# Tongji-MIC-Lab/TDVC

Hardware: AMD Instinct MI355X
Metric: 1080p P-frames/sec (encode + reconstruct, lambda=2048 config) (higher is better)
Workload: dtype f16; 1 GPU; 1x 1920x1080 (padded 1088x1920) 7-frame synthetic GOP (seed 1234), batch 1, P-frames coded in GOP order; gop=7, batch=1, parallelism=gop-sharded x1, weights=closed-form filler (no checkpoint ships)

## Files before the change

### include/tdvc_hip.h

```cpp
#ifndef TDVC_HIP_H
#define TDVC_HIP_H

#include <stdint.h>

#ifdef __cplusplus
extern "C" {
#endif

#define TDVC_OK 0
#define TDVC_EINVAL (-1)
#define TDVC_ENOSUP (-2)

typedef struct {
  void* p;
  int32_t N, H, W, C;
  int64_t sn;
  int32_t sp;
  int32_t dtype;
} tdvc_fmap;

enum { TDVC_F16 = 0, TDVC_F32 = 1 };
enum { TDVC_ACT_NONE = 0, TDVC_ACT_RELU = 1, TDVC_ACT_LRELU = 2, TDVC_ACT_CLAMP01 = 3, TDVC_ACT_SIGMOID = 4 };
enum { TDVC_GDN_NONE = 0, TDVC_GDN_FWD = 1, TDVC_GDN_INV = 2 };
enum { TDVC_OUT_NHWC = 0,
// ... 43 lines not shown
int tdvc_conv_plan(int cin, int kh, int kw, int stride);
int64_t tdvc_conv_packed_bytes(int cout, int cin, int ntaps, int ck);
int tdvc_pack_conv_weights(const float* w_oihw, int cout, int cin_real, int cin, int kh, int kw,
                           int ntaps, const int8_t* tap_dy, const int8_t* tap_dx, int ck, uint16_t* dst);
int tdvc_conv2d(const tdvc_conv_desc* d, void* stream);
int tdvc_conv_chan_sum_rows(const tdvc_conv_desc* d);
int tdvc_conv_flow_supported(const tdvc_conv_desc* d);
const char* tdvc_conv_select(const tdvc_conv_desc* d);
int tdvc_conv2d_f32(const tdvc_conv_desc* d, void* stream);

typedef struct {
  tdvc_fmap x, y;
  const void* w;
  const float* bias;
  int32_t act1; float slope1;
  int32_t act2; float slope2;
  int32_t add_input;
  tdvc_fmap res2;
} tdvc_conv_pair_desc;
int64_t tdvc_conv_pair_packed_bytes(void);
int tdvc_pack_conv_pair_weights(const float* w1_oihw, const float* w2_oihw, uint16_t* dst);
int tdvc_conv_pair_supported(const tdvc_conv_pair_desc* d);
int tdvc_conv_pair(const tdvc_conv_pair_desc* d, void* stream);

typedef struct {
  tdvc_fmap x, om, y;
  const void* w;
  const float* bias;
  int32_t groups;
  int32_t act; float slope; int32_t round_before_act;
  void* x_planar;
} tdvc_dcn_desc;
int tdvc_dcn_fused(const tdvc_dcn_desc* d, void* stream);

int tdvc_dcn_v2_forward_f32(const float* input, const float* weight, const float* bias,
                            const float* offset, const float* mask, float* output,
                            int B, int C, int H, int W, int Cout,
                            int kh, int kw, int sh, int sw, int ph, int pw, int dh, int dw,
                            int deformable_group, void* stream);
int tdvc_dcn_v2_backward_f32(const float* input, const float* weight, const float* bias,
                             const float* offset, const float* mask, const float* grad_output,
                             float* grad_input, float* grad_offset, float* grad_mask,
                             float* grad_weight, float* grad_bias, float* columns,
                             int B, int C, int H, int W, int Cout,
                             int kh, int kw, int sh, int sw, int ph, int pw, int dh, int dw,
                             int deformable_group, void* stream);
// ... 219 lines not shown
```

### tdvc_amd/_lib.py

```python
from __future__ import annotations

import ctypes as C
import os

_HERE = os.path.dirname(os.path.abspath(__file__))
LIB_PATH = os.path.join(_HERE, "libtdvc_hip.so")

MAX_TAPS = 49
F16, F32 = 0, 1
ACT_NONE, ACT_RELU, ACT_LRELU, ACT_CLAMP01, ACT_SIGMOID = 0, 1, 2, 3, 4
GDN_NONE, GDN_FWD, GDN_INV = 0, 1, 2
OUT_NHWC, OUT_SHUFFLE2, OUT_NCHW_F32 = 0, 1, 2


class FMapDesc(C.Structure):
    _fields_ = [("p", C.c_void_p), ("N", C.c_int32), ("H", C.c_int32), ("W", C.c_int32), ("C", C.c_int32),
                ("sn", C.c_int64), ("sp", C.c_int32), ("dtype", C.c_int32)]


class ConvDesc(C.Structure):
    _fields_ = [("x", FMapDesc), ("y", FMapDesc), ("w", C.c_void_p), ("bias", C.c_void_p),
                ("cout", C.c_int32), ("ntaps", C.c_int32),
                ("tap_dy", C.c_int8 * MAX_TAPS), ("tap_dx", C.c_int8 * MAX_TAPS),
                ("kh", C.c_int32), ("kw", C.c_int32), ("stride", C.c_int32), ("pad", C.c_int32),
                ("ck", C.c_int32), ("square_input", C.c_int32), ("gdn", C.c_int32),
                ("aux", FMapDesc), ("act", C.c_int32), ("slope", C.c_float),
                ("round_before_act", C.c_int32), ("res", FMapDesc), ("res2", FMapDesc), ("out_mode", C.c_int32), ("s2d", C.c_int32),
                ("bcast_T", C.c_int32), ("bcast_slope", C.c_float), ("chan_sum", C.c_void_p), ("flow", FMapDesc)]


class DcnDesc(C.Structure):
    _fields_ = [("x", FMapDesc), ("om", FMapDesc), ("y", FMapDesc), ("w", C.c_void_p), ("bias", C.c_void_p),
                ("groups", C.c_int32), ("act", C.c_int32), ("slope", C.c_float), ("round_before_act", C.c_int32), ("x_planar", C.c_void_p)]


class ConvPairDesc(C.Structure):
    _fields_ = [("x", FMapDesc), ("y", FMapDesc), ("w", C.c_void_p), ("bias", C.c_void_p), ("act1", C.c_int32), ("slope1", C.c_float),
                ("act2", C.c_int32), ("slope2", C.c_float), ("add_input", C.c_int32), ("res2", FMapDesc)]


class WgradReduceJob(C.Structure):
    _fields_ = [("work", C.c_void_p), ("bwork", C.c_void_p), ("row_off", C.c_void_p), ("chan_off", C.c_void_p), ("tap_off", C.c_void_p),
                ("bias_index", C.c_void_p), ("dw", C.c_void_p), ("db", C.c_void_p), ("scale", C.c_float),
                ("nworkers", C.c_int32), ("cow", C.c_int32), ("ciw", C.c_int32), ("ntaps", C.c_int32), ("cout", C.c_int32), ("cin", C.c_int32),
                ("wblocks", C.c_int32), ("nblocks", C.c_int32)]


_P = C.c_void_p
_FM = C.POINTER(FMapDesc)


class CdfTablesDesc(C.Structure):
    _fields_ = [("cdfs", _P), ("sizes", _P), ("offsets", _P), ("stride", C.c_int32), ("ncdfs", C.c_int32)]


class CdfTablesDevDesc(C.Structure):
    _fields_ = [("cdf16", _P), ("starts", _P), ("sizes", _P), ("offsets", _P), ("n16", C.c_int32), ("ncdfs", C.c_int32)]


class ArLoopDesc(C.Structure):
    _fields_ = [("y_hat", FMapDesc), ("params", FMapDesc), ("x1", FMapDesc), ("pc", FMapDesc), ("gp", FMapDesc),
# ... 75 lines not shown
    "tdvc_rans_encode_lanes_dev_ref": (_i, [_ENC, _CDF]),
    "tdvc_ar_last_loop_launches": (_i64, []),
    "tdvc_ssim_level_work_floats": (_i64, [_i] * 5),
    "tdvc_ssim_level": (_i, [_P, _P, _i, _i, _i, _i, _P, _i, _f, _f, _P, _P, _P, _i64, _P]),
    "tdvc_avgpool2_pad_f32": (_i, [_P, _i64, _i, _i, _P, _P]),
    "tdvc_ssim_level_backward": (_i, [_P, _P, _i, _i, _i, _i, _P, _i, _f, _f, _P, _P, _f, _P, _P, _P]),
    "tdvc_msssim_level_grads": (_i, [_P, _P, _P, _i, _i, _P, _P, _P, _P, _P]),
    "tdvc_dcn_col2im_work_floats": (_i64, [_i, _i, _i, _i]),
    "tdvc_dcn_col2im": (_i, [_FM, _FM, _FM, _i, _P, _FM, _P, _i64, _P]),
    "tdvc_dcn_col2im_det": (_i, [_FM, _FM, _FM, _i, _P, _FM, _P, _i64, _P, _P, _P, _i, _P]),
    "tdvc_dcn_far_apply": (_i, [_P, _P, _P, _i, _P, _P]),
    "tdvc_conv_wgrad_work_floats": (_i64, [_i] * 6),
    "tdvc_conv_wgrad": (_i, [_FM, _FM] + [_i] * 6 + [_P] * 5 + [_i, _f, _P, _P, _i64, _P]),
    "tdvc_conv_wgrad_bias": (_i, [_FM, _FM] + [_i] * 6 + [_P] * 5 + [_i, _f, _P, _P, _P, _P, _i64, _P]),
    "tdvc_conv_wgrad_partials": (_i, [_FM, _FM] + [_i] * 6 + [_P] * 5 + [_i, _f, _P, _P, _P, _P, _i64, C.POINTER(WgradReduceJob), _P]),
    "tdvc_wgrad_reduce_batch": (_i, [_P, _P, _i, _i, _P]),
    "tdvc_gdn_backward": (_i, [_FM, _FM, _FM, _i, _FM, _FM, _P]),
    "tdvc_mul2_accumulate": (_i, [_FM, _FM, _FM, _P]),
    "tdvc_dcn_fused": (_i, [C.POINTER(DcnDesc), _P]),
    "tdvc_conv_pair_packed_bytes": (_i64, []),
    "tdvc_pack_conv_pair_weights": (_i, [_P, _P, _P]),
    "tdvc_conv_pair_supported": (_i, [C.POINTER(ConvPairDesc)]),
    "tdvc_conv_pair": (_i, [C.POINTER(ConvPairDesc), _P]),
    "tdvc_dcn_v2_forward_f32": (_i, [_P] * 6 + [_i] * 14 + [_P]),
    "tdvc_dcn_v2_backward_f32": (_i, [_P] * 12 + [_i] * 14 + [_P]),
    "tdvc_nchw_to_fmap": (_i, [_P, _i, _FM, _P]),
    "tdvc_fmap_to_nchw": (_i, [_FM, _i, _P, _P]),
    "tdvc_scale_act_res": (_i, [_FM, _P, _i, _f, _FM, _f, _FM, _FM, _P]),
    "tdvc_add_flow": (_i, [_FM, _FM, _P]),
    "tdvc_bcast_add_act": (_i, [_FM, _FM, _i, _f, _P]),
    "tdvc_channel_sum": (_i, [_FM, _P, _i, _P]),
    "tdvc_se_gate": (_i, [_P, _i, _f, _i, _i, _i, _P, _P, _P, _P, _P, _P]),
    "tdvc_upsample2x": (_i, [_FM, _FM, _P]),
    "tdvc_avgpool2": (_i, [_FM, _FM, _P]),
    "tdvc_spynet_level_input": (_i, [_FM, _FM, _FM, _FM, _FM, _P]),
    "tdvc_resize_bilinear": (_i, [_FM, _FM, _P, _P]),
    "tdvc_avgpool_k_work_floats": (_i64, [_i, _i, _i, _i, _i]),
    "tdvc_avgpool_k": (_i, [_FM, _i, _P, _i, _i, _P, _i64, _P]),
    "tdvc_patch_match": (_i, [_P, _P, _i, _i, _i, _i, _P, _P]),
    "tdvc_match_gather": (_i, [_FM, _FM, _P, _i, _i, _i, _FM, _P]),
    "tdvc_eb_forward": (_i, [_FM, _P, _FM, _FM, _P, _P, _i, _P]),
    "tdvc_gc_forward": (_i, [_FM, _FM, _FM, _P, _P, _i, _P]),
    "tdvc_quantize": (_i, [_FM, _FM, _FM, _P]),
    "tdvc_rans_encode": (_i64, [_P, _P, _i64, _P, C.c_int32, _P, _P, _P, _i64]),
    "tdvc_rans_decode": (_i, [_P, _i64, _P, _i64, _P, C.c_int32, _P, _P, _P]),
    "tdvc_rans_encode_lanes": (_i64, [_P, _P, _i64, _i, _i, _P, C.c_int32, _P, _P, _P, _i64]),
# ... 40 lines not shown
```

### tdvc_amd/csrc/common.h

```cpp
#pragma once
#include <hip/hip_runtime.h>
#include <stdint.h>
#include <stdio.h>
#include <string.h>

#include "../../include/tdvc_hip.h"

typedef _Float16 half_t;
typedef _Float16 half8 __attribute__((ext_vector_type(8)));
typedef _Float16 half4 __attribute__((ext_vector_type(4)));
typedef _Float16 half2v __attribute__((ext_vector_type(2)));
typedef float f32x16 __attribute__((ext_vector_type(16)));
typedef float f32x4 __attribute__((ext_vector_type(4)));

void tdvc_set_error(const char* fmt, ...);
int tdvc_scratch_pages(const void** zeros, void** dump);

const int* tdvc_launch_predicate();
void tdvc_note_launch();
long tdvc_launch_count();
void tdvc_set_loop_launches(long n);
struct TdvcLoopLaunches {
  long start = tdvc_launch_count();
  ~TdvcLoopLaunches() { tdvc_set_loop_launches(tdvc_launch_count() - start); }
};
const int* tdvc_launch_predicate_images(int N);
#define TDVC_PREDICATE_RETURN(pred)                       \
  do {                                                    \
    if ((pred) != nullptr && *(pred) == 0) return;        \
  } while (0)

struct TdvcActiveImages { unsigned list; int count; };
__device__ __forceinline__ TdvcActiveImages tdvc_active_images(const int* flags, int nimg) {
  TdvcActiveImages a = {0xE4u, nimg};
  if (flags != nullptr) {
    a.list = 0u; a.count = 0;
    for (int i = 0; i < nimg; ++i)
      if (flags[i] != 0) { a.list |= (unsigned)i << (2 * a.count); ++a.count; }
  }
  return a;
}
__device__ __forceinline__ int tdvc_active_image(const TdvcActiveImages& a, int j) { return (int)((a.list >> (2 * j)) & 3u); }

#define TDVC_CHECK(cond, ...)            \
  do {                                   \
    if (!(cond)) {                       \
      tdvc_set_error(__VA_ARGS__);       \
      return TDVC_EINVAL;                \
// ... 66 lines not shown
```

### tdvc_amd/csrc/conv_dispatch.hip

```cpp
#include <stdlib.h>

#include "conv_common.h"

using convk::ConvParams;
bool conv_v2_eligible(const tdvc_conv_desc* d, int Ho, int Wo); int launch_conv_v2(const ConvParams& p, int cout_blocks, int N, hipStream_t st);
bool conv_v3_eligible(const tdvc_conv_desc* d, int Ho, int Wo); int launch_conv_v3(const ConvParams& p, int cout_blocks, int N, hipStream_t st);
bool conv_v5_eligible(const tdvc_conv_desc* d, int Ho, int Wo); int launch_conv_v5(const ConvParams& p, int cout_blocks, int N, hipStream_t st); int conv_v5_chan_sum_rows(int Ho, int Wo, int cout_blocks, int N);
bool conv_v7_eligible(const tdvc_conv_desc* d, const ConvParams& p, int Ho, int Wo); int launch_conv_v7(const ConvParams& p, int cout_blocks, int N, hipStream_t st);
bool conv_v9_eligible(const tdvc_conv_desc* d, int Ho, int Wo, bool v3_ok); int launch_conv_v9(const ConvParams& p, int ck8, int cout_tiles32, int N, hipStream_t st);
bool conv_v10_eligible(const tdvc_conv_desc* d, const ConvParams& p, int Ho, int Wo); int launch_conv_v10(const ConvParams& p, int cout_blocks, int N, hipStream_t st);
bool conv_v11_eligible(const tdvc_conv_desc* d, const ConvParams& p, int Ho, int Wo); int launch_conv_v11(const ConvParams& p, int cout_blocks, int N, hipStream_t st);
int conv_row_geometry(const tdvc_conv_desc* d, const ConvParams& p, int Ho, int Wo); int launch_conv_row(int geo, const ConvParams& p, int N, hipStream_t st);
bool conv_c8_eligible(const tdvc_conv_desc* d, const ConvParams& p, int Ho, int Wo); int launch_conv_c8(const ConvParams& p, int N, hipStream_t st);
bool conv_n16_eligible(const tdvc_conv_desc* d, int Ho, int Wo); int launch_conv_n16(const ConvParams& p, int N, hipStream_t st);
bool gdn128_eligible(const tdvc_conv_desc* d, const ConvParams& p, int Ho, int Wo); int launch_gdn128(const ConvParams& p, int N, hipStream_t st);
int conv_direct_lds_bytes(const tdvc_conv_desc* d);
int conv_cout_tiles(int cout);
int launch_conv_direct(const ConvParams& p, int ck8, int stride, int N, hipStream_t st);
int conv_f32_validate(const tdvc_conv_desc* d, int& Ho, int& Wo);

namespace {
const char* const kSwitchEnv[convk::SW_COUNT] = {nullptr, "TDVC_CONV_NO_V3", "TDVC_CONV_NO_V5", "TDVC_CONV_NO_V7", "TDVC_CONV_NO_V9", "TDVC_CONV_NO_V10",
                                                 "TDVC_CONV_NO_V11", "TDVC_CONV_NO_ROW", "TDVC_CONV_NO_C8", "TDVC_CONV_NO_N16", "TDVC_CONV_NO_GDN128", "TDVC_CONV_NO_HEAD3"};
int g_enabled[convk::SW_COUNT] = {1, 1, 1, 1, 1, 1, 1, 15, 1, 1, 1, 1};
// ... 221 lines not shown
  }
  ConvParams p;
  Pick k = {d, 0, 0, -1};
  if (const int rc = prepare(d, p, k.Ho, k.Wo)) return rc;
  p.reverse = query != LAUNCH ? 0 : next_walk_reverse();
  const Entry* e = select(k, p);
  const bool csum_ok = e && e->name == kNameV5 && k.cout_blocks() == 1 && p.simple == 2;
  if (query_rows) return csum_ok ? conv_v5_chan_sum_rows(k.Ho, k.Wo, 1, k.N()) : 0;
  if (query == QUERY_FLOW) return conv_flow_ok(d, e, p) && (!d->flow.p || flow_map_ok(d, k.Ho, k.Wo)) ? 1 : 0;
  TDVC_CHECK(!d->chan_sum || (csum_ok && (reinterpret_cast<uintptr_t>(d->chan_sum) & 15) == 0),
             "tdvc_conv2d: chan_sum on a conv whose kernel has no fused channel sum (tdvc_conv_chan_sum_rows() == 0) or unaligned");
  p.csum = d->chan_sum;
  if (!e) return TDVC_EINVAL;
  if (d->flow.p) {
    TDVC_CHECK(conv_flow_ok(d, e, p) && flow_map_ok(d, k.Ho, k.Wo), "%s", kFlowMsg);
    p.flow = to_dev(d->flow);
  }
  kernel_name(e, k, g_last_kernel);
  return e->launch(k, p, reinterpret_cast<hipStream_t>(stream));
}

}

extern "C" void tdvc_debug_set_conv_walk(int mode) { g_walk_mode = mode; }
extern "C" int tdvc_conv2d(const tdvc_conv_desc* d, void* stream) { return conv2d_impl(d, stream, LAUNCH); }
extern "C" int tdvc_conv_chan_sum_rows(const tdvc_conv_desc* d) { return conv2d_impl(d, nullptr, QUERY_ROWS); }
extern "C" int tdvc_conv_flow_supported(const tdvc_conv_desc* d) { return conv2d_impl(d, nullptr, QUERY_FLOW); }
extern "C" const char* tdvc_last_conv_kernel(void) { return g_last_kernel; }

extern "C" const char* tdvc_conv_select(const tdvc_conv_desc* d) {
  static thread_local char name[48];
  if (!d) { tdvc_set_error("tdvc_conv_select: null descriptor"); return nullptr; }
  if (d->x.dtype == TDVC_F32) {
    int Ho, Wo;
    if (d->flow.p) { tdvc_set_error("%s", kFlowMsg); return nullptr; }
    return conv_f32_validate(d, Ho, Wo) == TDVC_OK ? "conv_f32" : nullptr;
  }
  ConvParams p;
  Pick k = {d, 0, 0, -1};
  if (prepare(d, p, k.Ho, k.Wo) != TDVC_OK) return nullptr;
  const Entry* e = select(k, p);
  if (!e) return nullptr;
  if (d->flow.p && !(conv_flow_ok(d, e, p) && flow_map_ok(d, k.Ho, k.Wo))) { tdvc_set_error("%s", kFlowMsg); return nullptr; }
  kernel_name(e, k, name);
  return name;
}
// ... 1 lines not shown
```

### tdvc_amd/csrc/lib.cpp

```cpp
#include <hip/hip_runtime.h>
#include <stdarg.h>
#include <stddef.h>
#include <stdio.h>

#include <mutex>

#include "../../include/tdvc_hip.h"

static thread_local char g_err[512] = "";

void tdvc_set_error(const char* fmt, ...) {
  va_list ap;
  va_start(ap, fmt);
  vsnprintf(g_err, sizeof(g_err), fmt, ap);
  va_end(ap);
}

static_assert(sizeof(tdvc_cdf_tables) == 32 && offsetof(tdvc_cdf_tables, ncdfs) == 28, "tdvc_cdf_tables layout");
static_assert(sizeof(tdvc_cdf_tables_dev) == 40 && offsetof(tdvc_cdf_tables_dev, ncdfs) == 36, "tdvc_cdf_tables_dev layout");
static_assert(sizeof(tdvc_ar_loop) == 272 && offsetof(tdvc_ar_loop, sym_dev) == 264, "tdvc_ar_loop layout");
static_assert(sizeof(tdvc_lanes_enc) == 104 && offsetof(tdvc_lanes_enc, info) == 96, "tdvc_lanes_enc layout");

extern "C" int tdvc_abi_version(void) { return 13; }
extern "C" const char* tdvc_last_error(void) { return g_err; }

static thread_local const int* g_pred = nullptr;
static thread_local int g_pred_taken = 0, g_pred_last = 0;
static thread_local const int* g_pred_img = nullptr;
static thread_local int g_pred_img_n = 0;

extern "C" int tdvc_set_predicate(const int* flag) {
  if (reinterpret_cast<uintptr_t>(flag) & 3) { tdvc_set_error("tdvc_set_predicate: flag must be 4-byte aligned"); return TDVC_EINVAL; }
  if (flag && g_pred_img) { tdvc_set_error("tdvc_set_predicate: a per-image predicate is set (clear it first)"); return TDVC_EINVAL; }
  g_pred = flag;
  return TDVC_OK;
}
extern "C" int tdvc_set_predicate_images(const int* flags, int n) {
  if (!flags || n == 0) { g_pred_img = nullptr; g_pred_img_n = 0; return TDVC_OK; }
  if (reinterpret_cast<uintptr_t>(flags) & 3) { tdvc_set_error("tdvc_set_predicate_images: flags must be 4-byte aligned"); return TDVC_EINVAL; }
  if (n < 1 || n > TDVC_MAX_PREDICATE_IMAGES) { tdvc_set_error("tdvc_set_predicate_images: 1 <= n <= %d images, got %d", TDVC_MAX_PREDICATE_IMAGES, n); return TDVC_EINVAL; }
  if (g_pred) { tdvc_set_error("tdvc_set_predicate_images: a launch predicate is set (clear it first)"); return TDVC_EINVAL; }
  g_pred_img = flags; g_pred_img_n = n;
  return TDVC_OK;
}
const int* tdvc_launch_predicate_images(int N) {
  if (!g_pred_img || N != g_pred_img_n) return nullptr;
// ... 52 lines not shown
```

### tdvc_amd/model/modules.py

```python
from __future__ import annotations

import torch
import torch.nn as nn

from .. import ops
from ..ops import ACT_LRELU, ACT_NONE, ACT_RELU, FM
from .ring import SlotRing


class PackCache:

    def _pk(self, key, fn):
        c = self.__dict__.setdefault("_packed", {})
        if key not in c:
            c[key] = fn()
        return c[key]


def _dev(m: nn.Module):
    return next(m.parameters()).device


def pk_conv(owner: PackCache, name: str, conv: nn.Module, **kw) -> ops.PackedConv:
    def build():
# ... 248 lines not shown
    def run(self, offset: FM, feats: FM, out: FM) -> FM:
        ref = feats.ch(64, 64)
        dcn_out = feats.ch(128, 64)
        self.dconv.run(ref, offset, dcn_out, act=ACT_LRELU, slope=0.1)
        perm = list(range(64, 128)) + list(range(0, 64))
        pc = self._pk("conv", lambda: ops.pack_conv(self.conv.weight, self.conv.bias, stride=1, pad=1, cin_perm=perm,
                                                    device=self.conv.weight.device))
        o2 = ops.conv(feats.ch(64, 128), pc, act=ACT_LRELU, slope=0.1)
        return run_stack(self.recon_layer, o2, out=out, res2=dcn_out)


class Bottleneck3D(nn.Module):
    def __init__(self):
        super().__init__()
        self.conv1 = nn.Conv3d(64, 64, (1, 3, 3), padding=(0, 1, 1))
        self.spatial_conv3d = nn.Conv3d(64, 64, (1, 3, 3), padding=(0, 1, 1))
        self.temporal_conv3d = nn.Conv3d(64, 64, (3, 1, 1), stride=(3, 1, 1), bias=False)
        self.conv3 = nn.Conv3d(64, 64, (1, 3, 3), padding=(0, 1, 1))


LOOPFILTER_PAIR = True
LOOPFILTER_BCAST = True
LOOPFILTER_REUSE = True
LOOPFILTER_RING = 9


class LoopFilterReuse:

    __slots__ = ("key", "ring", "A", "S", "F", "flags", "usable", "log")

    def __init__(self, key, slots):
        self.key, self.ring, self.usable, self.log = key, SlotRing(slots), None, []
        self.A = self.S = self.F = self.flags = None


class LoopFilter(nn.Module, PackCache):

    def __init__(self):
        super().__init__()
        self.conv01 = nn.Conv2d(3, 64, 3, 1, 1)
        self.conv02 = nn.Conv2d(64, 64, 3, 1, 1)
        self.conv1 = nn.Conv3d(64, 64, (1, 3, 3), padding=(0, 1, 1))
        self.layer1 = Bottleneck3D()
        self.attn = SELayer(64)
        self.feat_fusion = nn.Conv2d(256, 64, 1, 1)

    def _slices(self, name, conv, src: FM, dst: FM, res_buf: FM | None = None, **kw):
        pc = pk_conv(self, name, conv)
        for b in range(src.N):
            ops.conv(src.as_slices(b, 4, 64), pc, out=dst.as_slices(b, 4, 64),
                     res=res_buf.as_slices(b, 4, 64) if res_buf is not None else None, **kw)

    def run(self, xt: FM, refs8: FM, out: FM, then: tuple | None = None) -> FM:
        if (LOOPFILTER_REUSE and LOOPFILTER_PAIR and LOOPFILTER_BCAST and not self.training and ops.TAPE is None and ops.PROFILE is None
                and not xt.f32 and not refs8.f32 and xt.H * xt.W >= 8192 and ops.conv_pair_supported(xt.as_slices(0, 4, 64))):
            r = self._run_reuse(xt, refs8, out, then)
            if r is not None:
                return r
        return self._run_plain(xt, refs8, out, then)

    def reuse_state(self) -> LoopFilterReuse | None:
        return self.__dict__.get("_packed", {}).get("lf_reuse")

    def _run_reuse(self, xt: FM, refs8: FM, out: FM, then: tuple | None = None) -> FM | None:
        B, H, W = xt.N, xt.H, xt.W
        dev = xt.t.device
        key = (dev.index, ops._stream().value, B, H, W)
        cache = self.__dict__.setdefault("_packed", {})
        st = cache.get("lf_reuse")
        if st is None or st.key != key or st.ring.slots != LOOPFILTER_RING:
            st = cache["lf_reuse"] = LoopFilterReuse(key, LOOPFILTER_RING)
        if st.usable is False:
            return None
        try:
            return self._reuse_call(st, xt, refs8, out, then)
        except BaseException:
            cache.pop("lf_reuse", None)
            raise

    def _reuse_call(self, st: LoopFilterReuse, xt: FM, refs8: FM, out: FM, then: tuple | None = None) -> FM | None:
        B, H, W = xt.N, xt.H, xt.W
        dev = xt.t.device
# ... 15 lines not shown
        pp_a = self._pk("pair_c02_c1", lambda: ops.pack_conv_pair(self.conv02.weight, self.conv02.bias,
                                                                   self.conv1.weight.view(64, 64, 3, 3), self.conv1.bias))
        pp_b = self._pk("pair_b1_bs", lambda: ops.pack_conv_pair(l1.conv1.weight.view(64, 64, 3, 3), l1.conv1.bias,
                                                                  l1.spatial_conv3d.weight.view(64, 64, 3, 3), l1.spatial_conv3d.bias))
        log = []
        for b in range(B):
            frames = refs8.batch(4 * b + 1, 3)
            ops.frames_changed(frames, st.F.batch(b * R + p, 3), st.flags[b, :3], force)
            with ops.predicate_images(st.flags[b, :3]) as lg:
                t = ops.conv(frames, p01, **lr)
                ops.conv_pair(t, pp_a, out=win(st.A, b, 0, 3), act1=ACT_NONE, act2=ACT_LRELU, slope2=0.1, add_input=False)
            log += lg
            ops.conv(xt.as_slices(b, 4, 64).batch(3, 1), pc1, out=win(st.A, b, 3, 1), **lr)
            with ops.predicate_images(st.flags[b, :4]) as lg:
                ops.conv_pair(win(st.A, b, 0, 4), pp_b, out=win(st.S, b, 0, 4), act1=ACT_LRELU, slope1=0.1, act2=ACT_NONE, add_input=False)
            log += lg
        st.log = list(log)
        if not all(log):
            st.usable = False
            st.A = st.S = st.F = st.flags = None
            return None
        st.usable = True
        st.ring.commit()
        s = FM.empty(B, H, W, 256, device=dev)
        ops.conv(st.S.ch(64 * p, 192), pk_conv(self, "bt", l1.temporal_conv3d), out=s.ch(0, 64), bcast_T=4, bcast_slope=0.1,
                 res=st.S.ch(64 * p, 64))
        o = FM.empty(B, H, W, 256, device=dev)
        pc3 = pk_conv(self, "b3", l1.conv3)
        for b in range(B):
            ops.conv(s.as_slices(b, 4, 64), pc3, out=o.as_slices(b, 4, 64), res=win(st.A, b, 0, 4))
        sums = []
        f = ops.conv(o, pk_conv(self, "ff", self.feat_fusion), chan_sum=sums, **lr)
        return self.attn.run(f, out=out, res=xt.ch(192, 64), sums=sums, then=then)

    def _run_plain(self, xt: FM, refs8: FM, out: FM, then: tuple | None = None) -> FM:
        B, H, W = xt.N, xt.H, xt.W
        dev = xt.t.device
        lr = dict(act=ACT_LRELU, slope=0.1)
        p01, p02 = pk_conv(self, "c01", self.conv01), pk_conv(self, "c02", self.conv02)
        a = FM.empty(B, H, W, 256, device=dev)
        fuse = LOOPFILTER_PAIR and ops.conv_pair_supported(a.as_slices(0, 4, 64).batch(0, 3))
        if fuse:
            pp = self._pk("pair_c02_c1", lambda: ops.pack_conv_pair(self.conv02.weight, self.conv02.bias,
                                                                     self.conv1.weight.view(64, 64, 3, 3), self.conv1.bias))
            pc1 = pk_conv(self, "c1", self.conv1)
        for b in range(B):
            t = ops.conv(refs8.batch(4 * b + 1, 3), p01, **lr)
            if fuse:
                ops.conv_pair(t, pp, out=a.as_slices(b, 4, 64).batch(0, 3), act1=ACT_NONE, act2=ACT_LRELU, slope2=0.1, add_input=False)
                ops.conv(xt.as_slices(b, 4, 64).batch(3, 1), pc1, out=a.as_slices(b, 4, 64).batch(3, 1), **lr)
            else:
                ops.conv(t, p02, out=xt.as_slices(b, 4, 64).batch(0, 3))
        if not fuse:
            self._slices("c1", self.conv1, xt, a, **lr)
        l1 = self.layer1
        bf = FM.empty(B, H, W, 256, device=dev)
        s = FM.empty(B, H, W, 256, device=dev)
        if LOOPFILTER_PAIR and ops.conv_pair_supported(a.as_slices(0, 4, 64), s.as_slices(0, 4, 64)):
            pp = self._pk("pair_b1_bs", lambda: ops.pack_conv_pair(l1.conv1.weight.view(64, 64, 3, 3), l1.conv1.bias,
                                                                    l1.spatial_conv3d.weight.view(64, 64, 3, 3), l1.spatial_conv3d.bias))
            for b in range(B):
                ops.conv_pair(a.as_slices(b, 4, 64), pp, out=s.as_slices(b, 4, 64), act1=ACT_LRELU, slope1=0.1, act2=ACT_NONE,
                              add_input=False)
        else:
            self._slices("b1", l1.conv1, a, bf, **lr)
            self._slices("bs", l1.spatial_conv3d, bf, s)
        if ops.TAPE is None and LOOPFILTER_BCAST and H * W >= 8192:
            ops.conv(s.ch(0, 192), pk_conv(self, "bt", l1.temporal_conv3d), out=s.ch(0, 64), bcast_T=4, bcast_slope=0.1)
        else:
            tm = ops.conv(s.ch(0, 192), pk_conv(self, "bt", l1.temporal_conv3d))
            if ops.TAPE is not None:
                s = ops.clone(s)
            ops.bcast_add_act(s, tm, 4, 0.1)
        o = bf if ops.TAPE is None else FM.empty(B, H, W, 256, device=dev)
        self._slices("b3", l1.conv3, s, o, res_buf=a)
        sums = []
        f = ops.conv(o, pk_conv(self, "ff", self.feat_fusion), chan_sum=sums, **lr)
        return self.attn.run(f, out=out, res=xt.ch(192, 64), sums=sums, then=then)


class FeatureExtract(nn.Module, PackCache):

    def __init__(self, cin, mid, nblocks):
        super().__init__()
        self.conv_first = nn.Conv2d(cin, mid, 3, 1, 1)
        self.body = res_stack(nblocks, mid)
        self.conv_last = nn.Conv2d(mid, mid, 3, 1, 1)

    def run(self, x: FM, out: FM | None = None) -> FM:
# ... 106 lines not shown
```

### tdvc_amd/ops.py

```python
from __future__ import annotations

import ctypes as C
from dataclasses import dataclass

import numpy as np
import torch

from . import _lib as L
from . import convpack
from ._lib import (ACT_CLAMP01, ACT_LRELU, ACT_NONE, ACT_RELU, GDN_FWD, GDN_INV, GDN_NONE, OUT_NCHW_F32,
                   OUT_NHWC, OUT_SHUFFLE2)


_raw_stream = torch._C._cuda_getCurrentRawStream
_cur_dev = torch._C._cuda_getDevice
FORCE_STREAM = None
FORCE_KEEP = None


def _stream():
    if FORCE_STREAM is not None:
        return C.c_void_p(FORCE_STREAM)
    return C.c_void_p(_raw_stream(_cur_dev()))

# ... 542 lines not shown


def conv_pair(x: FM, pp: PackedConvPair, out: FM | None = None, act1=ACT_RELU, slope1=0.0, act2=ACT_NONE, slope2=0.0,
              add_input=True, res2: FM | None = None) -> FM:
    if TAPE is not None:
        raise L.TdvcHipError("conv_pair: inference only (the intermediate map is not kept for the backward pass)")
    if out is None:
        out = FM.empty(x.N, x.H, x.W, 64, device=x.t.device)
    d = _pair_desc(x, pp, out, act1, slope1, act2, slope2, add_input, res2)
    if PROFILE is not None:
        e0, e1 = torch.cuda.Event(enable_timing=True), torch.cuda.Event(enable_timing=True)
        e0.record()
        L.check(L.lib().tdvc_conv_pair(C.byref(d), _stream()), "conv_pair")
        e1.record()
        fl = 2 * 2.0 * x.N * x.H * x.W * 64 * 64 * 9
        PROFILE.append(dict(kernel="conv_pair", shape=f"2x(3x3 s1 64->64) @{x.H}x{x.W}", e0=e0, e1=e1, flops=fl, flops_real=fl,
                            bytes=2.0 * x.N * x.H * x.W * 128))
        return out
    L.check(L.lib().tdvc_conv_pair(C.byref(d), _stream()), "conv_pair")
    _log_predicated()
    return out


def act_backward(g: FM, y: FM, act, slope=0.0, res: FM | None = None, out: FM | None = None) -> FM:
    out = g if out is None else out
    dg, dy, do = g.desc(), y.desc(), out.desc()
    dr = res.desc() if res is not None else None
    L.check(L.lib().tdvc_act_backward(C.byref(dg), C.byref(dy), C.byref(dr) if dr is not None else None, act, slope, C.byref(do), _stream()),
            "act_backward")
    return out


def pixel_unshuffle(y: FM, out: FM | None = None) -> FM:
    if out is None:
        out = FM.empty(y.N, y.H // 2, y.W // 2, 4 * y.C, dtype=y.t.dtype, device=y.t.device)
    dy, do = y.desc(), out.desc()
    L.check(L.lib().tdvc_pixel_unshuffle(C.byref(dy), C.byref(do), _stream()), "pixel_unshuffle")
    return out


def _dgrad_conv(pc: PackedConv, g_channels: int, x_channels: int) -> PackedConv:
    if pc.dgrad is None:
        o = pc.orig
        tb0 = dict(g_channels=g_channels, x_channels=x_channels, taps=o["taps"], pad=o["pad"], stride=o["stride"], shuffle=pc.shuffle,
                   cin_perm=o["cin_perm"], device=pc.w.device)
        rows = x_channels * (4 if o["stride"] == 2 else 1)
# ... 873 lines not shown
```

Measured before the change: 51.69 frames/s.

## Fuse loop-filter temporal 1x1 conv, broadcast-add, and conv3 into one streaming kernel

Adds a dedicated HIP kernel that, per 32-column strip, computes the 1x1 temporal conv (192->64), broadcasts it onto the four slices with leaky ReLU, then runs the 3x3 conv3 with residual add, all staged in LDS through a row ring buffer. Loader waves issue global-to-LDS row prefetches while compute waves do the 3x3 MFMA work. It replaces the separate bcast temporal conv plus the per-batch conv3 launches in both the reuse and plain loop-filter paths, removing the intermediate map round trip through global memory. It adds a large, intricate kernel with a hand-tuned wait schedule and new support checks (no temporal bias, disjoint buffers, size floor).

```diff
diff --git a/include/tdvc_hip.h b/include/tdvc_hip.h
--- a/include/tdvc_hip.h
+++ b/include/tdvc_hip.h
@@ -89,6 +89,19 @@
 int tdvc_pack_conv_pair_weights(const float* w1_oihw, const float* w2_oihw, uint16_t* dst);
 int tdvc_conv_pair_supported(const tdvc_conv_pair_desc* d);
 int tdvc_conv_pair(const tdvc_conv_pair_desc* d, void* stream);
+
+typedef struct {
+  tdvc_fmap s, a, y;
+  int32_t nslices;
+  int32_t slice_stride;
+  const void* wt;
+  const float* bias_t;
+  const void* w3;
+  const float* bias3;
+  float slope;
+} tdvc_lf_tail_desc;
+int tdvc_lf_tail_supported(const tdvc_lf_tail_desc* d);
+int tdvc_lf_tail(const tdvc_lf_tail_desc* d, void* stream);
 
 typedef struct {
   tdvc_fmap x, om, y;
diff --git a/tdvc_amd/_lib.py b/tdvc_amd/_lib.py
--- a/tdvc_amd/_lib.py
+++ b/tdvc_amd/_lib.py
@@ -37,6 +37,11 @@
 class ConvPairDesc(C.Structure):
     _fields_ = [("x", FMapDesc), ("y", FMapDesc), ("w", C.c_void_p), ("bias", C.c_void_p), ("act1", C.c_int32), ("slope1", C.c_float),
                 ("act2", C.c_int32), ("slope2", C.c_float), ("add_input", C.c_int32), ("res2", FMapDesc)]
+
+
+class LfTailDesc(C.Structure):
+    _fields_ = [("s", FMapDesc), ("a", FMapDesc), ("y", FMapDesc), ("nslices", C.c_int32), ("slice_stride", C.c_int32),
+                ("wt", C.c_void_p), ("bias_t", C.c_void_p), ("w3", C.c_void_p), ("bias3", C.c_void_p), ("slope", C.c_float)]
 
 
 class WgradReduceJob(C.Structure):
@@ -158,6 +163,8 @@
     "tdvc_pack_conv_pair_weights": (_i, [_P, _P, _P]),
     "tdvc_conv_pair_supported": (_i, [C.POINTER(ConvPairDesc)]),
     "tdvc_conv_pair": (_i, [C.POINTER(ConvPairDesc), _P]),
+    "tdvc_lf_tail_supported": (_i, [C.POINTER(LfTailDesc)]),
+    "tdvc_lf_tail": (_i, [C.POINTER(LfTailDesc), _P]),
     "tdvc_dcn_v2_forward_f32": (_i, [_P] * 6 + [_i] * 14 + [_P]),
     "tdvc_dcn_v2_backward_f32": (_i, [_P] * 12 + [_i] * 14 + [_P]),
     "tdvc_nchw_to_fmap": (_i, [_P, _i, _FM, _P]),
diff --git a/tdvc_amd/csrc/common.h b/tdvc_amd/csrc/common.h
--- a/tdvc_amd/csrc/common.h
+++ b/tdvc_amd/csrc/common.h
@@ -24,6 +24,7 @@
   long start = tdvc_launch_count();
   ~TdvcLoopLaunches() { tdvc_set_loop_launches(tdvc_launch_count() - start); }
 };
+void tdvc_conv_walk_advance(int launches);
 const int* tdvc_launch_predicate_images(int N);
 #define TDVC_PREDICATE_RETURN(pred)                       \
   do {                                                    \
diff --git a/tdvc_amd/csrc/conv_dispatch.hip b/tdvc_amd/csrc/conv_dispatch.hip
--- a/tdvc_amd/csrc/conv_dispatch.hip
+++ b/tdvc_amd/csrc/conv_dispatch.hip
@@ -267,6 +267,8 @@
 
 }
 
+void tdvc_conv_walk_advance(int launches) { g_walk_parity += (unsigned)launches; }
+
 extern "C" void tdvc_debug_set_conv_walk(int mode) { g_walk_mode = mode; }
 extern "C" int tdvc_conv2d(const tdvc_conv_desc* d, void* stream) { return conv2d_impl(d, stream, LAUNCH); }
 extern "C" int tdvc_conv_chan_sum_rows(const tdvc_conv_desc* d) { return conv2d_impl(d, nullptr, QUERY_ROWS); }
diff --git a/tdvc_amd/csrc/lf_tail.hip b/tdvc_amd/csrc/lf_tail.hip
--- /dev/null
+++ b/tdvc_amd/csrc/lf_tail.hip
@@ -0,0 +1,370 @@
+#include <type_traits>
+
+#include "conv_dma.h"
+
+using convk::glds16;
+using convk::raw_barrier;
+
+namespace {
+
+constexpr int LT_SW = 32, LT_RPX = LT_SW + 2, LT_PXB = 512, LT_PIECES = 17, LT_ROWB = LT_PIECES * 1024;
+constexpr int LT_XRING = 6, LT_PF = 5;
+constexpr int LT_SROW = LT_SW * LT_PXB;
+constexpr int LT_TPS = 144, LT_TROW = LT_RPX * LT_TPS;
+constexpr int LT_X0 = 0, LT_S0 = LT_XRING * LT_ROWB, LT_T0 = LT_S0 + 2 * LT_SROW, LT_B0 = LT_T0 + 2 * LT_TROW, LT_LDS = LT_B0 + 256;
+constexpr int LT_NTHR = 512;
+static_assert(LT_RPX * LT_PXB == LT_ROWB, "a ring row is exactly 17 pieces");
+static_assert(LT_PF >= 5 && LT_PF < LT_XRING, "ring conditions");
+static_assert((LT_T0 % 16) == 0 && LT_LDS <= 160 * 1024, "LDS");
+
+struct TailParams {
+  const half_t* s; long s_sn; int s_sp;
+  const half_t* a; long a_sn; int a_sp;
+  half_t* y; long y_sn; int y_sp;
+  const half_t* wt;
+  const half_t* w3;
+  const float* bias3;
+  const half_t* zeros;
+  half_t* dump;
+  int N, H, W, strips;
+  float slope;
+  float tzero;
+};
+
+__device__ __forceinline__ int lt_f(int q) { return (q & 12) | ((q & 1) << 1) | ((q >> 1) & 1); }
+__device__ __forceinline__ int lt_sigma(int r) { return r < 4 ? 2 * r : (r >= 12 ? 2 * r - 16 : 2 * r - 7); }
+__device__ __forceinline__ int lt_g(int q) { return (q >> 1) & 7; }
+
+__global__ __launch_bounds__(LT_NTHR, 1) void lf_tail_kernel(const TailParams p) {
+  extern __shared__ __attribute__((aligned(1024))) unsigned char smem[];
+  const unsigned lds0 = static_cast<unsigned>(reinterpret_cast<uintptr_t>(smem));
+  const int tid = threadIdx.x, lane = tid & 63;
+  const int wave = __builtin_amdgcn_readfirstlane(tid >> 6);
+  const bool loader = wave < 4;
+  const int wq = wave & 3;
+  const int cg = wave & 3, ip = wave >> 2;
+  const int r16 = lane & 15, kb = lane >> 4;
+
+  const int nwg = (int)gridDim.x, b = (int)blockIdx.x;
+  int pos_slot = b;
+  if ((nwg & 7) == 0) pos_slot = (b & 7) * (nwg >> 3) + (b >> 3);
+  const long allrows = (long)p.N * p.strips * p.H;
+  const long run_begin = allrows * pos_slot / nwg, run_end = allrows * (pos_slot + 1) / nwg;
+
+  half8 wf[18];
+  {
+    const int co = 16 * cg + r16;
+    const half_t* wb = p.w3 + ((long)(co >> 5) * 2 * 18 * 64 + (kb & 1) * 32 + (co & 31)) * 8 + (long)(kb >> 1) * 512;
+#pragma unroll
+    for (int tap = 0; tap < 9; ++tap)
+#pragma unroll
+      for (int kc = 0; kc < 2; ++kc) wf[tap * 2 + kc] = *reinterpret_cast<const half8*>(wb + ((long)kc * 18 + tap * 2) * 512);
+  }
+  if (tid < 64) reinterpret_cast<float*>(smem + LT_B0)[tid] = p.bias3[tid];
+  const int boff = LT_B0 + (16 * cg + 4 * kb) * 4;
+
+  int foff[3];
+#pragma unroll
+  for (int dx = 0; dx < 3; ++dx) {
+    const int q = dx + lt_sigma(r16);
+    foff[dx] = q * LT_PXB + ((kb ^ lt_f(q)) << 4);
+  }
+  int doff[2];
+#pragma unroll
+  for (int cb = 0; cb < 2; ++cb) {
+    const int q = 16 * cb + lt_sigma(r16), c = 16 * ip + 2 * cg + (kb >> 1);
+    doff[cb] = q * LT_PXB + ((c ^ lt_g(q)) << 4) + 8 * (kb & 1);
+  }
+  const int a2_pos = tid & 31, a2_q = tid >> 5;
+  const int a2_slot = a2_pos ^ lt_f(a2_q);
+  const int a2_x = a2_q * LT_PXB + a2_pos * 16, a2_t = a2_q * LT_TPS + (a2_slot & 7) * 16;
+  const bool a2_third = tid >= LT_NTHR - 64;
+  const int a2_t3 = (a2_q + 18) * LT_TPS + ((a2_pos ^ lt_f(a2_q - 14)) & 7) * 16;
+
+  auto run = [&](auto LOADERc) __attribute__((always_inline)) {
+  constexpr bool LOADER = decltype(LOADERc)::value;
+  const int dq = 2 * wq + (lane >> 5);
+  int soff[2];
+#pragma unroll
+  for (int j = 0; j < 2; ++j) {
+    const int q = dq + 8 * j;
+    soff[j] = q * p.s_sp + (((lane & 31) ^ lt_f(q)) << 3);
+  }
+  const int mt = wq & 1, nt = wq >> 1;
+  const int a1_q = min(32 * nt + (lane & 31), LT_RPX - 1), a1_hh = lane >> 5;
+  const bool a1_ok = 32 * nt + (lane & 31) < LT_RPX;
+  const int a1_x = a1_q * LT_PXB + ((a1_hh ^ lt_f(a1_q)) << 4);
+  const int a1_t = a1_q * LT_TPS + (32 * mt + 4 * a1_hh) * 2;
+  half8 tw[LOADER ? 12 : 1];
+  if constexpr (LOADER) {
+#pragma unroll
+    for (int m = 0; m < 12; ++m) tw[m] = *reinterpret_cast<const half8*>(p.wt + ((long)(mt * 12 + m) * 64 + lane) * 8);
+  }
+  const int s_t = tid & 255;
+  int s_px[4], s_co[4];
+#pragma unroll
+  for (int j = 0; j < 4; ++j) {
+    const int it = s_t + 256 * j;
+    s_px[j] = it >> 5;
+    s_co[j] = ((it & 31) ^ lt_g(it >> 5)) << 3;
+  }
+
+  f32x4 acc[3][2][2];
+  half8 r1v[4] = {};
+
+  for (long pos = run_begin; pos < run_end;) {
+    const int sid = (int)(pos / p.H);
+    const int ra = (int)(pos - (long)sid * p.H), rb = (int)min((long)p.H, ra + (run_end - pos));
+    const int rows = rb - ra;
+    pos += rows;
+    const int n = sid / p.strips, strip = sid - n * p.strips;
+    const int c0 = strip * LT_SW;
+    const int last_in = rows + 1;
+
+    unsigned colok = 0;
+#pragma unroll
+    for (int j = 0; j < 5; ++j) {
+      const int col = c0 - 1 + dq + 8 * j;
+      colok |= (col >= 0 && col < p.W) ? (1u << j) : 0u;
+    }
+    bool s_ok[4];
+    int y_lo[4], r_lo[4];
+#pragma unroll
+    for (int j = 0; j < 4; ++j) {
+      const int col = c0 + s_px[j], colc = min(col, p.W - 1);
+      s_ok[j] = col < p.W;
+      y_lo[j] = col * p.y_sp + s_co[j];
+      r_lo[j] = colc * p.a_sp + s_co[j];
+    }
+    const half_t* const yimg = p.y + (long)n * p.y_sn;
+    const half_t* const rimg = p.a + (long)n * p.a_sn;
+    const long yrow_stride = (long)p.W * p.y_sp, rrow_stride = (long)p.W * p.a_sp, xrow_stride = (long)p.W * p.s_sp;
+    const half_t* const xcol = p.s + (long)n * p.s_sn + (long)(c0 - 1) * p.s_sp;
+#pragma unroll
+    for (int s3 = 0; s3 < 3; ++s3)
+#pragma unroll
+      for (int cb = 0; cb < 2; ++cb)
+#pragma unroll
+        for (int jj = 0; jj < 2; ++jj) acc[s3][cb][jj] = f32x4{0.f, 0.f, 0.f, 0.f};
+
+    auto issue_row = [&](int kk) __attribute__((always_inline)) -> int {
+      const int row = ra - 1 + kk;
+      const bool rowok = row >= 0 && row < p.H;
+      const half_t* base = xcol + row * xrow_stride;
+      const unsigned dst = lds0 + LT_X0 + (__builtin_amdgcn_readfirstlane(kk) % LT_XRING) * LT_ROWB;
+      const unsigned okb = rowok ? colok : 0u;
+#pragma nounroll
+      for (int j = 0; j < 4; ++j) {
+        const half_t* src = base + (long)(16 * (j >> 1)) * p.s_sp + soff[j & 1];
+        glds16(((okb >> j) & 1u) ? src : p.zeros, dst + (wq + 4 * j) * 1024);
+      }
+      if (wq == 0) {
+        glds16(((okb >> 4) & 1u) ? base + (long)32 * p.s_sp + soff[0] : p.zeros, dst + (LT_PIECES - 1) * 1024);
+        return 5;
+      }
+      return 4;
+    };
+    auto land_wait = [&](int nvm) __attribute__((always_inline)) {
+      if (!nvm) { asm volatile("s_waitcnt vmcnt(0)" ::: "memory"); return; }
+      if (wq == 0) asm volatile("s_waitcnt vmcnt(10)" ::: "memory");
+      else asm volatile("s_waitcnt vmcnt(8)" ::: "memory");
+    };
+    auto phase_a1 = [&](int kk) __attribute__((always_inline)) {
+      if constexpr (LOADER) {
+        const unsigned char* xb = smem + LT_X0 + (__builtin_amdgcn_readfirstlane(kk) % LT_XRING) * LT_ROWB;
+        unsigned char* tb = smem + LT_T0 + (kk & 1) * LT_TROW;
+        f32x16 t;
+#pragma unroll
+        for (int i = 0; i < 16; ++i) t[i] = 0.f;
+        half8 bf[2];
+        bf[0] = *reinterpret_cast<const half8*>(xb + a1_x);
+#pragma unroll
+        for (int m = 0; m < 12; ++m) {
+          if (m + 1 < 12) bf[(m + 1) & 1] = *reinterpret_cast<const half8*>(xb + (a1_x ^ ((m + 1) << 5)));
+          t = __builtin_amdgcn_mfma_f32_32x32x16_f16(tw[m], bf[m & 1], t, 0, 0, 0);
+        }
+        if (a1_ok) {
+#pragma unroll
+          for (int g = 0; g < 4; ++g) {
+            const float v0 = t[4 * g] + p.tzero, v1 = t[4 * g + 1] + p.tzero, v2 = t[4 * g + 2] + p.tzero, v3 = t[4 * g + 3] + p.tzero;
+            *reinterpret_cast<half4*>(tb + a1_t + 16 * g) = half4{(half_t)v0, (half_t)v1, (half_t)v2, (half_t)v3};
+          }
+        }
+      }
+    };
+    auto phase_a2 = [&](int kk) __attribute__((always_inline)) {
+      unsigned char* xb = smem + LT_X0 + (__builtin_amdgcn_readfirstlane(kk) % LT_XRING) * LT_ROWB;
+      const unsigned char* tb = smem + LT_T0 + (kk & 1) * LT_TROW;
+      auto item = [&](int qadd, int toff) __attribute__((always_inline)) {
+        unsigned char* xp = xb + a2_x + qadd * LT_PXB;
+        const half8 xs = *reinterpret_cast<const half8*>(xp);
+        const half8 v = *reinterpret_cast<const half8*>(tb + toff);
+        half8 o;
+#pragma unroll
+        for (int j = 0; j < 8; ++j) {
+          const float s = (float)xs[j] + (float)v[j];
+          o[j] = (half_t)(s > 0.f ? s : s * p.slope);
+        }
+        *reinterpret_cast<half8*>(xp) = o;
+      };
+      item(0, a2_t);
+      item(16, a2_t + 16 * LT_TPS);
+      if (!LOADER && a2_third) item(18, a2_t3);
+    };
+
+    if constexpr (LOADER) {
+#pragma unroll
+      for (int kk = 0; kk < LT_PF; ++kk)
+        if (kk <= last_in) issue_row(kk);
+    }
+    asm volatile("s_waitcnt vmcnt(0)" ::: "memory");
+    raw_barrier();
+    phase_a1(0);
+    raw_barrier();
+    phase_a1(1);
+    phase_a2(0);
+    raw_barrier();
+
+    const int K = rows + 3;
+    auto step = [&](auto PHc, auto FULLc, int k) __attribute__((always_inline)) {
+      constexpr int PH = decltype(PHc)::value;
+      constexpr bool FULL = decltype(FULLc)::value;
+      constexpr int SD = (PH + 1) % 3;
+      if constexpr (!LOADER) {
+        const int srow = ra + k - 3;
+        if (FULL || (srow >= ra && srow < rb)) {
+          const unsigned char* sb = smem + LT_S0 + ((k - 1) & 1) * LT_SROW;
+          half_t* const yrow = const_cast<half_t*>(yimg) + srow * yrow_stride;
+#pragma unroll
+          for (int j = 0; j < 4; ++j) {
+            half8 yv = *reinterpret_cast<const half8*>(sb + (s_t + 256 * j) * 16);
+            yv = yv + r1v[j];
+            *reinterpret_cast<half8*>(s_ok[j] ? yrow + y_lo[j] : p.dump + (s_t + 256 * j) * 8) = yv;
+          }
+        }
+        const int nrow = srow + 1;
+        const bool rok = FULL || (nrow >= ra && nrow < rb);
+        const half_t* const rrow = rimg + (rok ? nrow : ra) * rrow_stride;
+#pragma unroll
+        for (int j = 0; j < 4; ++j) r1v[j] = *reinterpret_cast<const half8*>(rrow + r_lo[j]);
+        if (FULL || k + 1 <= last_in) phase_a2(k + 1);
+      } else {
+        if (FULL || k + 2 <= last_in) phase_a1(k + 2);
+      }
+      int nvm = 0;
+      if (FULL || k <= last_in) {
+        const unsigned char* xb = smem + LT_X0 + (__builtin_amdgcn_readfirstlane(k) % LT_XRING) * LT_ROWB;
+        half8 fb[2][2];
+        auto load_group = [&](int gi, int buf) __attribute__((always_inline)) {
+          const int jj = gi / 6, g = gi - 6 * jj, kc = g / 3, dx = g - 3 * kc;
+          const unsigned char* b0 = xb + (foff[dx] ^ ((8 * (2 * ip + jj) + 4 * kc) << 4));
+#pragma unroll
+          for (int cb = 0; cb < 2; ++cb) fb[buf][cb] = *reinterpret_cast<const half8*>(b0 + cb * 16 * LT_PXB);
+        };
+        const f32x4 bias4 = *reinterpret_cast<const f32x4*>(smem + boff);
+        load_group(0, 0);
+#pragma unroll
+        for (int gi = 0; gi < 12; ++gi) {
+          const int jj = gi / 6, g = gi - 6 * jj, kc = g / 3, dx = g - 3 * kc;
+          if (gi + 1 < 12) load_group(gi + 1, (gi + 1) & 1);
+#pragma unroll
+          for (int dyo = 0; dyo < 3; ++dyo) {
+            const int dy = 2 - dyo;
+            const int slot = (PH + 3 - dy) % 3;
+#pragma unroll
+            for (int cb = 0; cb < 2; ++cb) {
+              const bool first = dy == 0 && g == 0;
+              acc[slot][cb][jj] = __builtin_amdgcn_mfma_f32_16x16x32_f16(wf[(dy * 3 + dx) * 2 + kc], fb[gi & 1][cb],
+                                                                         first ? bias4 : acc[slot][cb][jj], 0, 0, 0);
+            }
+          }
+        }
+        if (LOADER && k + LT_PF <= last_in) nvm = issue_row(k + LT_PF);
+        {
+          unsigned char* sb = smem + LT_S0 + (k & 1) * LT_SROW;
+#pragma unroll
+          for (int cb = 0; cb < 2; ++cb)
+#pragma unroll
+            for (int jj = 0; jj < 2; ++jj) {
+              const f32x4 v = acc[SD][cb][jj];
+              const half4 h = {(half_t)v[0], (half_t)v[1], (half_t)v[2], (half_t)v[3]};
+              *reinterpret_cast<half4*>(sb + doff[cb] + 128 * jj) = h;
+            }
+        }
+      }
+      if constexpr (LOADER) {
+        if (FULL || k + 1 <= last_in) phase_a2(k + 1);
+        land_wait(nvm);
+      }
+      raw_barrier();
+    };
+    auto steps_of = [&](auto FULLc, int k0, int kend) __attribute__((always_inline)) {
+      step(std::integral_constant<int, 0>{}, FULLc, k0);
+      if (k0 + 1 < kend) step(std::integral_constant<int, 1>{}, FULLc, k0 + 1);
+      if (k0 + 2 < kend) step(std::integral_constant<int, 2>{}, FULLc, k0 + 2);
+    };
+    int k = 0;
+    for (; k < 3; k += 3) steps_of(std::false_type{}, k, min(3, K));
+    for (; k + 2 + 2 <= last_in; k += 3) steps_of(std::true_type{}, k, k + 3);
+    for (; k < K; k += 3) steps_of(std::false_type{}, k, K);
+  }
+  };
+  if (loader) run(std::true_type{});
+  else run(std::false_type{});
+}
+
+bool lt_disjoint(const tdvc_fmap& x, const tdvc_fmap& y) {
+  const uintptr_t xa = (uintptr_t)x.p, ya = (uintptr_t)y.p;
+  const uintptr_t xe = xa + 2 * ((uintptr_t)(x.N - 1) * x.sn + ((uintptr_t)x.H * x.W - 1) * x.sp + x.C);
+  const uintptr_t ye = ya + 2 * ((uintptr_t)(y.N - 1) * y.sn + ((uintptr_t)y.H * y.W - 1) * y.sp + y.C);
+  return !(xa < ye && ya < xe);
+}
+
+const char* lt_refusal(const tdvc_lf_tail_desc* d) {
+  if (!d) return "null descriptor";
+  const tdvc_fmap &s = d->s, &a = d->a, &y = d->y;
+  if (d->nslices != 4 || d->slice_stride != 64) return "four slices at channel offsets 0, 64, 128, 192";
+  if (s.dtype != TDVC_F16 || a.dtype != TDVC_F16 || y.dtype != TDVC_F16) return "s, a and y must be fp16 maps";
+  if (!fmap_ok16(s) || !fmap_ok16(a) || !fmap_ok16(y)) return "s, a and y must be 16-byte aligned maps with channels and strides in multiples of 8";
+  if (s.C != 256 || a.C != 256 || y.C != 256) return "s, a and y must have 4 x 64 channels";
+  if (a.N != s.N || a.H != s.H || a.W != s.W || y.N != s.N || y.H != s.H || y.W != s.W) return "s / a / y geometry mismatch";
+  if ((long)s.H * s.W < convk::LARGE_MAP_PIXELS || s.H < 16) return "the map is under the floor (8192 pixels, 16 rows)";
+  const long px = (long)s.H * s.W;
+  if (px * s.sp >= (1L << 31) || px * a.sp >= (1L << 31) || px * y.sp >= (1L << 31)) return "element offsets within an image must fit 32 bits";
+  if (!d->wt || !d->w3 || !d->bias3 || !aligned16(d->wt) || !aligned16(d->w3) || ((uintptr_t)d->bias3 & 3)) return "weights / conv3 bias missing or misaligned";
+  if (d->bias_t) return "the temporal conv must have no bias (zero padding is applied behind it)";
+  if (!lt_disjoint(s, y) || !lt_disjoint(a, y)) return "y overlaps s or a (the kernel is out of place)";
+  return nullptr;
+}
+
+}
+
+extern "C" int tdvc_lf_tail_supported(const tdvc_lf_tail_desc* d) { return lt_refusal(d) ? 0 : 1; }
+
+extern "C" int tdvc_lf_tail(const tdvc_lf_tail_desc* d, void* stream) {
+  if (const char* why = lt_refusal(d)) {
+    tdvc_set_error("tdvc_lf_tail: %s", why);
+    return TDVC_EINVAL;
+  }
+  const void* zeros = nullptr;
+  void* dump = nullptr;
+  if (const int zrc = tdvc_scratch_pages(&zeros, &dump)) return zrc;
+  TailParams q;
+  q.s = reinterpret_cast<const half_t*>(d->s.p); q.s_sn = d->s.sn; q.s_sp = d->s.sp;
+  q.a = reinterpret_cast<const half_t*>(d->a.p); q.a_sn = d->a.sn; q.a_sp = d->a.sp;
+  q.y = reinterpret_cast<half_t*>(d->y.p); q.y_sn = d->y.sn; q.y_sp = d->y.sp;
+  q.wt = reinterpret_cast<const half_t*>(d->wt);
+  q.w3 = reinterpret_cast<const half_t*>(d->w3);
+  q.bias3 = d->bias3;
+  q.zeros = reinterpret_cast<const half_t*>(zeros);
+  q.dump = reinterpret_cast<half_t*>(dump);
+  q.N = d->s.N; q.H = d->s.H; q.W = d->s.W;
+  q.strips = (q.W + LT_SW - 1) / LT_SW;
+  q.slope = d->slope;
+  q.tzero = 0.f;
+  const long allrows = (long)q.N * q.strips * q.H;
+  const int grid = allrows < 256 ? (int)allrows : 256;
+  const int rc = convk::launch_big_lds<&lf_tail_kernel>("tdvc_lf_tail", LT_LDS, dim3(grid), dim3(LT_NTHR), LT_LDS, reinterpret_cast<hipStream_t>(stream), q);
+  if (rc == TDVC_OK) tdvc_conv_walk_advance(1 + q.N);
+  return rc;
+}
diff --git a/tdvc_amd/csrc/lib.cpp b/tdvc_amd/csrc/lib.cpp
--- a/tdvc_amd/csrc/lib.cpp
+++ b/tdvc_amd/csrc/lib.cpp
@@ -19,9 +19,10 @@
 static_assert(sizeof(tdvc_cdf_tables) == 32 && offsetof(tdvc_cdf_tables, ncdfs) == 28, "tdvc_cdf_tables layout");
 static_assert(sizeof(tdvc_cdf_tables_dev) == 40 && offsetof(tdvc_cdf_tables_dev, ncdfs) == 36, "tdvc_cdf_tables_dev layout");
 static_assert(sizeof(tdvc_ar_loop) == 272 && offsetof(tdvc_ar_loop, sym_dev) == 264, "tdvc_ar_loop layout");
+static_assert(sizeof(tdvc_lf_tail_desc) == 168 && offsetof(tdvc_lf_tail_desc, slope) == 160, "tdvc_lf_tail_desc layout");
 static_assert(sizeof(tdvc_lanes_enc) == 104 && offsetof(tdvc_lanes_enc, info) == 96, "tdvc_lanes_enc layout");
 
-extern "C" int tdvc_abi_version(void) { return 13; }
+extern "C" int tdvc_abi_version(void) { return 14; }
 extern "C" const char* tdvc_last_error(void) { return g_err; }
 
 static thread_local const int* g_pred = nullptr;
diff --git a/tdvc_amd/model/modules.py b/tdvc_amd/model/modules.py
--- a/tdvc_amd/model/modules.py
+++ b/tdvc_amd/model/modules.py
@@ -294,6 +294,7 @@
 LOOPFILTER_PAIR = True
 LOOPFILTER_BCAST = True
 LOOPFILTER_REUSE = True
+LOOPFILTER_TAIL = True
 LOOPFILTER_RING = 9
 
 
@@ -330,6 +331,10 @@
             if r is not None:
                 return r
         return self._run_plain(xt, refs8, out, then)
+
+    def _tail_ok(self, S: FM, A: FM, o: FM) -> bool:
+        return (LOOPFILTER_TAIL and LOOPFILTER_BCAST and not self.training and ops.TAPE is None and ops.PROFILE is None
+                and self.layer1.temporal_conv3d.bias is None and ops.lf_tail_supported(S, A, o))
 
     def reuse_state(self) -> LoopFilterReuse | None:
         return self.__dict__.get("_packed", {}).get("lf_reuse")
@@ -391,13 +396,15 @@
             return None
         st.usable = True
         st.ring.commit()
-        s = FM.empty(B, H, W, 256, device=dev)
-        ops.conv(st.S.ch(64 * p, 192), pk_conv(self, "bt", l1.temporal_conv3d), out=s.ch(0, 64), bcast_T=4, bcast_slope=0.1,
-                 res=st.S.ch(64 * p, 64))
         o = FM.empty(B, H, W, 256, device=dev)
-        pc3 = pk_conv(self, "b3", l1.conv3)
-        for b in range(B):
-            ops.conv(s.as_slices(b, 4, 64), pc3, out=o.as_slices(b, 4, 64), res=win(st.A, b, 0, 4))
+        pct, pc3 = pk_conv(self, "bt", l1.temporal_conv3d), pk_conv(self, "b3", l1.conv3)
+        if self._tail_ok(st.S.ch(64 * p, 256), st.A.ch(64 * p, 256), o):
+            ops.lf_tail(st.S.ch(64 * p, 256), st.A.ch(64 * p, 256), pct, pc3, out=o, slope=0.1)
+        else:
+            s = FM.empty(B, H, W, 256, device=dev)
+            ops.conv(st.S.ch(64 * p, 192), pct, out=s.ch(0, 64), bcast_T=4, bcast_slope=0.1, res=st.S.ch(64 * p, 64))
+            for b in range(B):
+                ops.conv(s.as_slices(b, 4, 64), pc3, out=o.as_slices(b, 4, 64), res=win(st.A, b, 0, 4))
         sums = []
         f = ops.conv(o, pk_conv(self, "ff", self.feat_fusion), chan_sum=sums, **lr)
         return self.attn.run(f, out=out, res=xt.ch(192, 64), sums=sums, then=then)
@@ -434,6 +441,11 @@
         else:
             self._slices("b1", l1.conv1, a, bf, **lr)
             self._slices("bs", l1.spatial_conv3d, bf, s)
+        if self._tail_ok(s, a, bf):
+            ops.lf_tail(s, a, pk_conv(self, "bt", l1.temporal_conv3d), pk_conv(self, "b3", l1.conv3), out=bf, slope=0.1)
+            sums = []
+            f = ops.conv(bf, pk_conv(self, "ff", self.feat_fusion), chan_sum=sums, **lr)
+            return self.attn.run(f, out=out, res=xt.ch(192, 64), sums=sums, then=then)
         if ops.TAPE is None and LOOPFILTER_BCAST and H * W >= 8192:
             ops.conv(s.ch(0, 192), pk_conv(self, "bt", l1.temporal_conv3d), out=s.ch(0, 64), bcast_T=4, bcast_slope=0.1)
         else:
diff --git a/tdvc_amd/ops.py b/tdvc_amd/ops.py
--- a/tdvc_amd/ops.py
+++ b/tdvc_amd/ops.py
@@ -588,6 +588,36 @@
     return out
 
 
+def _lf_tail_desc(S: FM, A: FM, out: FM, pct: PackedConv | None, pc3: PackedConv | None, slope: float):
+    d = L.LfTailDesc()
+    d.s, d.a, d.y = S.desc(), A.desc(), out.desc()
+    d.nslices, d.slice_stride = 4, 64
+    if pct is None:
+        d.wt, d.bias_t, d.w3, d.bias3 = 16, None, 16, 16
+    else:
+        d.wt, d.bias_t = pct.w.data_ptr(), (None if pct.bsrc is None else pct.bias.data_ptr())
+        d.w3, d.bias3 = pc3.w.data_ptr(), pc3.bias.data_ptr()
+    d.slope = float(slope)
+    return d
+
+
+def lf_tail_supported(S: FM, A: FM, out: FM) -> bool:
+    if TAPE is not None or S.f32 or A.f32 or out.f32:
+        return False
+    return bool(L.lib().tdvc_lf_tail_supported(C.byref(_lf_tail_desc(S, A, out, None, None, 0.0))))
+
+
+def lf_tail(S: FM, A: FM, pct: PackedConv, pc3: PackedConv, out: FM, slope: float = 0.1) -> FM:
+    if TAPE is not None:
+        raise L.TdvcHipError("lf_tail: inference only (the intermediate map is not kept for the backward pass)")
+    if (pct.cin, pct.cout, pct.kh, pct.kw, pct.ck) != (192, 64, 1, 1, 32) or (pc3.cin, pc3.cout, pc3.kh, pc3.kw, pc3.ck, pc3.stride, pc3.pad) != (64, 64, 3, 3, 32, 1, 1):
+        raise L.TdvcHipError("lf_tail: needs the 1x1 192 -> 64 temporal conv and the 3x3 64 -> 64 conv, both packed with ck = 32")
+    d = _lf_tail_desc(S, A, out, pct, pc3, slope)
+    L.check(L.lib().tdvc_lf_tail(C.byref(d), _stream()), "lf_tail")
+    _log_predicated()
+    return out
+
+
 def act_backward(g: FM, y: FM, act, slope=0.0, res: FM | None = None, out: FM | None = None) -> FM:
     out = g if out is None else out
     dg, dy, do = g.desc(), y.desc(), out.desc()
```

Result: faster. 52.43 frames/s, median of 6 (+1.4%).
